# peterWon/LVI-ExC

Measured on AMD Instinct MI355X. Metric: M residual+Jacobian evals/s per GN iter, higher is better.
Workload: dtype f64; 1 GPU; config4-full-LVI: 1000000 surfel + 200000 IMU samples (gyro+accel blocks) + 49992 ORB reprojection blocks, 25023 knots @ dt=0.02; step = residuals + analytic Jacobians + Huber + J^T J/J^T r assembly (no linear solve); n_tangent=155259, bandwidth=179, n_border=52, tracks=orb, parallelism=sequence-per-gpu x1, allreduce_transport=none (one sequence)

## Files before the change

lvi-exc_amd/csrc/lvx_eval.hip:

```cpp
#include <algorithm>
#include <cmath>
#include <cstring>
#include <functional>
#include <numeric>
#include <cstdlib>

#include <thread>
#include "lvx_ctx.h"

namespace lvx {

#define LVX_PW 4
struct Keys { int k0, k1, lm; };
LVX_HD bool same(const Keys& a, const Keys& b) { return a.k0 == b.k0 && a.k1 == b.k1 && a.lm == b.lm; }

struct Cal { ImuCal imu; SensorCal lidar, cam; const double* rho; };
__device__ __forceinline__ Cal load_cal(const DevCommon& cm) {
  const double* s = cm.state + 7 * (size_t)cm.N;
  Cal c;
  c.imu.tau = s[7]; c.imu.roll = s[8]; c.imu.pitch = s[9]; c.imu.ba = load_v3(s + 10); c.imu.bg = load_v3(s + 13);
  c.lidar.q = load_q(s + 16); c.lidar.p = load_v3(s + 20); c.lidar.tau = s[23];
  c.cam.q = load_q(s + 24); c.cam.p = load_v3(s + 28); c.cam.tau = s[31];
  c.rho = s + 32;
  return c;
}

struct HubShared { PoseEval A; int ok; double M[6][24]; };

struct GyroFam {
  enum { NC = GYRO_NC, NR = GYRO_NR, USES_HUB = 0, FAM = LVX_FAM_GYRO, KEYS = 1 };
  int n; const double* t; const double* m3; const int* perm; double weight, huber;
  __device__ void make_hub(const DevCommon&, const SplineRef&, const Cal&, HubShared*) const {}
  __device__ int eval(const DevCommon& cm, const SplineRef& sp, const Cal& cal, const HubShared&, int si, double r[NR], double (*J)[NC], Keys& k) const {
    k.k1 = 0; k.lm = 0;
    return gyro_residual<true>(sp, cal.imu, t[si], load_v3(m3 + 3 * (size_t)si), weight, &k.k0, r, J);
  }
  __device__ int col(int c, const Keys& k, int N) const { return gyro_col(c, k.k0, N); }
};
struct AccelFam {
  enum { NC = ACC_NC, NR = ACC_NR, USES_HUB = 0, FAM = LVX_FAM_ACCEL, KEYS = 1 };
  int n; const double* t; const double* m3; const int* perm; double weight, huber;
// ... 312 lines not shown
    const int l0 = seg_l0[sg];
    const int l1 = sg + 1 < nseg ? seg_l0[sg + 1] : 64;
    const int rb = l0 * NR, re = l1 * NR;
    const int* cp = &cpos[sg * NC];
#pragma unroll
    for (int i = 0; i < ITER; ++i) {
      const int p = tid + NT * i;
      if (p < NP) {
        const int a = code[i] & 0xff, b = code[i] >> 8;
        const int pa = cp[a], pb = cp[b];
        if (pa == LVX_DEAD || pb == LVX_DEAD) continue;
        const double* ja = &Jt[a * TS];
        const double* jb = &Jt[b * TS];
        double acc = 0.0;
        for (int row = rb; row < re; ++row) acc += ja[row] * jb[row];
        if (a != b && pa == pb) acc *= 2.0;
        add_H(cm, pa, pb, acc, rep);
      } else if (p < NP + NC) {
        const int c = p - NP;
        const int pc = cp[c];
        if (pc == LVX_DEAD) continue;
        const double* jc = &Jt[c * TS];
        double acc = 0.0;
        for (int row = rb; row < re; ++row) acc += jc[row] * rs[row];
        add_g(cm, pc, acc, rep);
      }
    }
  }
}

__device__ void hub_eval_thread(const DevCommon& cm, double t_map, int want_surf, int want_cs, HubShared* hubs, int s) {
  if (s > 1) return;
  if ((s == 0 && !want_surf) || (s == 1 && !want_cs)) { hubs[s].ok = 0; return; }
  const SplineRef sp{cm.t0, cm.dt, cm.N, cm.state, cm.state + 3 * (size_t)cm.N};
  const Cal cal = load_cal(cm);
  const bool tl = s == 0 ? (cm.locks & LVX_LOCK_LIDAR_TAU) != 0 : (cm.locks & LVX_LOCK_CAM_TAU) != 0;
  const double tau = s == 0 ? cal.lidar.tau : cal.cam.tau;
  double s1[1][2]; hub_spans(t_map, tl, cm.sensor_mto, s1);
  Segs sg; KnotRef kh; hubs[s].ok = 0;
  if (!build_segments(sp, s1, 1, &sg)) return;
  if (!seg_lookup(sp, sg, t_map + tau, &kh)) return;
  if (!(tl ? pose_eval<true>(sp, kh, &hubs[s].A) : pose_eval<true, true>(sp, kh, &hubs[s].A))) { hubs[s].ok = -RES_NONUNIT; return; }
  hub_matrix(hubs[s].A, hubs[s].M);
  hubs[s].ok = 1;
}
__device__ __forceinline__ void state_prepass_block(const DevCommon& cm, So3Pre* tab, int nblk_tab, double t_map, int want_surf, int want_cs, HubShared* hubs, int blk) {
  if (blk >= nblk_tab) { hub_eval_thread(cm, t_map, want_surf, want_cs, hubs, threadIdx.x); return; }
  const int k = blk * blockDim.x + threadIdx.x;
  if (k >= cm.N) return;
  const double* so3 = cm.state + 3 * (size_t)cm.N;
  So3Pre e;
  if (k + 1 < cm.N) so3_pre(load_q(so3 + 4 * (size_t)k), load_q(so3 + 4 * (size_t)(k + 1)), &e);
  else { e.Om = mk(0, 0, 0); e.on = 0.0; e.Jri = m3_identity(); e.c3 = 1.0 / 12.0; e.ok = 1; }
  tab[k] = e;
}

struct Aux { int wid, xk, lm; const PreWin* pw; };
struct GyroAcc {
  enum { PMAJ = 1 };
  enum { NK = 12, NG = 3, NR = 3, HUB = -1, KPK = 3, LVO = 3, WS = 1, GL = 32, SKIP_GG = 0, SECONDARY = 0, LB = 64, NCP = 15, USE_PRE = 1, OCC = 1, FAM = LVX_FAM_GYRO };
  __device__ static constexpr int jm(int c) { return c; }
  int n; const double* t; const double* m3; const int* perm; double weight, huber;
  __device__ int eval(const DevCommon& cm, const SplineRef& sp, const Cal& cal, const HubShared*, int si, double r[NR], double (*J)[NCP], int& key, Aux& aux) const {
    return gyro_residual<true, true>(sp, cal.imu, t[si], load_v3(m3 + 3 * (size_t)si), weight, &key, r, J, aux.pw);
  }
  __device__ static int klv(int c) { return 6 * (c / 3) + 3 + c % 3; }
  __device__ static int gcol(int g, int N, int nt) { return 6 * N + 5 + g; }
  __device__ void put(const DevCommon& cm, const HubShared*, int si, bool valid, int key, const double (*J)[NCP]) const {
    if (!valid) { put_skipped(cm, FAM, perm[si]); return; }
    put_record<NR, GYRO_NC>(cm, FAM, perm[si], key, -1, -1, [&](int a, int c) { return J[a][c]; });
  }
};
#ifndef LVX_SURF_WS
#define LVX_SURF_WS 3
#endif
template <bool TAU> struct SurfAccT {
  enum { DEPG = LVX_SURF_WS >= 3 ? 3 : 0 };
// ... 1308 lines not shown
  const HubShared* hub = ((const HubShared*)cm.hubs) + set;
  if (hub->ok != 1) return;
  __shared__ double M[6][24];
  __shared__ int hrow[24];
  if (threadIdx.x < 144) M[threadIdx.x / 24][threadIdx.x % 24] = hub->M[threadIdx.x / 24][threadIdx.x % 24];
  if (threadIdx.x < 24) { const int o = cm.ord[6 * (hub->A.k.i0 + threadIdx.x / 6) + threadIdx.x % 6]; hrow[threadIdx.x] = (o != LVX_DEAD && o < 0) ? -1 - o : -1; }
  __syncthreads();
  const int j = blk * blockDim.x + threadIdx.x;
  double P[6];
  bool any = false;
  if (j < cm.nb) {
#pragma unroll
    for (int p = 0; p < 6; ++p) { P[p] = cm.Bd[(size_t)(cm.nbd_solve + 6 * set + p) * cm.nb + j]; any = any || P[p] != 0.0; }
  }
  const bool far = store && j < cm.nb && (j < cm.hub_lo || j >= cm.hub_hi);
  if (any || far) {
#pragma unroll
    for (int c = 0; c < 24; ++c) {
      if (hrow[c] < 0) continue;
      double s = 0.0;
#pragma unroll
      for (int p = 0; p < 6; ++p) s += M[p][c] * P[p];
      double* dst = &cm.Bd[(size_t)hrow[c] * cm.nb + j];
      if (far) *dst = any ? s : 0.0; else *dst += s;
    }
  }
  __syncthreads();
}
__global__ __launch_bounds__(256) void k_fold_border_rows(DevCommon cm, int set, int store) { fold_border_rows_block(cm, set, (int)blockIdx.x, store != 0); }
__device__ __forceinline__ void fold_border_dense_block(const DevCommon& cm) {
  extern __shared__ double Cf[];
  const int n = cm.nbd;
  double* g = Cf + n * n;
  for (int e0 = threadIdx.x; e0 < n * n; e0 += 8 * 256) {
    double v[8];
#pragma unroll
    for (int q = 0; q < 8; ++q) { const int e = e0 + 256 * q; if (e < n * n) { const int a = e / n, b = e % n; v[q] = a >= b ? cm.C[(size_t)a * n + b] : cm.C[(size_t)b * n + a]; } }
#pragma unroll
    for (int q = 0; q < 8; ++q) { const int e = e0 + 256 * q; if (e < n * n) Cf[e] = v[q]; }
  }
  for (int e = threadIdx.x; e < n; e += 256) g[e] = cm.gc[e];
  __syncthreads();
  for (int set = 0; set < 2; ++set) {
    const HubShared* hub = ((const HubShared*)cm.hubs) + set;
    if (hub->ok != 1) continue;
    __shared__ double M[6][24];
    __shared__ int hrow[24];
    if (threadIdx.x < 144) M[threadIdx.x / 24][threadIdx.x % 24] = hub->M[threadIdx.x / 24][threadIdx.x % 24];
    if (threadIdx.x < 24) { const int o = cm.ord[6 * (hub->A.k.i0 + threadIdx.x / 6) + threadIdx.x % 6]; hrow[threadIdx.x] = (o != LVX_DEAD && o < 0) ? -1 - o : -1; }
    __syncthreads();
    const int p0 = cm.nbd_solve + 6 * set;
    for (int e = threadIdx.x; e < 24 * n; e += 256) {
      const int c = e / n, col = e % n;
      if (hrow[c] < 0) continue;
      double s = 0.0;
      for (int p = 0; p < 6; ++p) s += M[p][c] * Cf[(p0 + p) * n + col];
      Cf[hrow[c] * n + col] += s;
    }
    if (threadIdx.x < 24 && hrow[threadIdx.x] >= 0) { double s = 0.0; for (int p = 0; p < 6; ++p) s += M[p][threadIdx.x] * g[p0 + p]; g[hrow[threadIdx.x]] += s; }
    __syncthreads();
    for (int e = threadIdx.x; e < 24 * n; e += 256) {
      const int c = e / n, row = e % n;
      if (hrow[c] < 0) continue;
      double s = 0.0;
      for (int p = 0; p < 6; ++p) s += Cf[row * n + p0 + p] * M[p][c];
      Cf[row * n + hrow[c]] += s;
    }
    __syncthreads();
  }
  for (int e = threadIdx.x; e < n * n; e += 256) { const int a = e / n, b = e % n; if (a >= b) cm.C[(size_t)a * n + b] = Cf[e]; }
  for (int e = threadIdx.x; e < n; e += 256) cm.gc[e] = g[e];
}

__global__ __launch_bounds__(256) void k_fold_border_dense(DevCommon cm) { fold_border_dense_block(cm); }

__device__ __forceinline__ double strided_sum(const double* p, size_t stride, int n) {
  double s = 0.0;
  for (int r0 = 0; r0 < n; r0 += 16) {
    double v[16];
#pragma unroll
    for (int q = 0; q < 16; ++q) v[q] = r0 + q < n ? p[(size_t)(r0 + q) * stride] : 0.0;
#pragma unroll
    for (int q = 0; q < 16; ++q) s += v[q];
  }
  return s;
}
__device__ __forceinline__ void fold_replicas_block(const DevCommon& cm, int blk) {
  const int n2 = cm.nbd * cm.nbd;
  const int i = blk * blockDim.x + threadIdx.x;
  if (cm.what & LVX_EVAL_NORMAL_EQ) {
    if (i < n2) cm.C[i] = strided_sum(cm.C + i, (size_t)n2, cm.nrep);
    if (i < cm.nbd) cm.gc[i] = strided_sum(cm.gc + i, (size_t)cm.nbd, cm.nrep);
  }
  if (i == 0) cm.cost[0] = strided_sum(cm.cost, 1, cm.nrep);
}
__global__ void k_fold_replicas(DevCommon cm) { fold_replicas_block(cm, (int)blockIdx.x); }
__global__ __launch_bounds__(256) void k_fold_all(DevCommon cm, int n_rep, int n_rows, int set0, int store0, int set1, int store1, int* ticket) {
  __shared__ int s_last;
  const int b = blockIdx.x;
  if (b < n_rep) {
    fold_replicas_block(cm, b);
    __threadfence();
    __syncthreads();
    if (threadIdx.x == 0) { const int t = atomicAdd(ticket, 1); s_last = t == n_rep - 1; if (s_last) *ticket = 0; }
    __syncthreads();
    if (!s_last) return;
    __threadfence();
    fold_border_dense_block(cm);
    return;
  }
  const int r = b - n_rep;
  fold_border_rows_block(cm, set0, r, store0 != 0);
  if (set1 >= 0) fold_border_rows_block(cm, set1, r, store1 != 0);
}
int fail(lvx_ctx* ctx, int code, const std::string& msg) { if (ctx) ctx->last_error = msg; return code; }

int dev_alloc(lvx_ctx* ctx, DevBuf& b, size_t bytes) {
  if (bytes == 0) bytes = 8;
  if (b.p && b.bytes >= bytes) return LVX_OK;
  if (b.p) { (void)hipFree(b.p); b.p = nullptr; b.bytes = 0; }
  if (hipMalloc(&b.p, bytes) != hipSuccess) { b.p = nullptr; return fail(ctx, LVX_E_ALLOC, "hipMalloc failed"); }
  b.bytes = bytes;
  return LVX_OK;
}
int upload(lvx_ctx* ctx, DevBuf& b, const void* src, size_t bytes) {
  int rc = dev_alloc(ctx, b, bytes);
  if (rc) return rc;
  if (bytes) LVX_HIP(ctx, hipMemcpyAsync(b.p, src, bytes, hipMemcpyHostToDevice, ctx->stream));
  return LVX_OK;
}
int upload_tmp(lvx_ctx* ctx, DevBuf& b, const void* src, size_t bytes) {
  int rc = upload(ctx, b, src, bytes);
  if (rc) return rc;
  LVX_HIP(ctx, hipStreamSynchronize(ctx->stream));
  return LVX_OK;
}

namespace {

template <class F> void par_for(size_t n, F&& fn) {
  const unsigned hw = std::thread::hardware_concurrency();
  const size_t nt = n < 200000 ? 1 : std::min<size_t>(8, hw ? hw : 1);
  if (nt <= 1) { fn((size_t)0, n); return; }
  std::vector<std::thread> th;
  const size_t per = (n + nt - 1) / nt;
  for (size_t t = 1; t < nt; ++t) { const size_t a = std::min(n, t * per), b = std::min(n, a + per); if (a < b) th.emplace_back([&fn, a, b] { fn(a, b); }); }
// ... 637 lines not shown
        double* col = bc.Hb + (size_t)j * bc.ld;
        if (!(bc.ld & 1)) {
          uint4* c4 = (uint4*)col;
          for (int e = (beg >> 1) + l16; e < (len >> 1); e += 16) c4[e] = make_uint4(0u, 0u, 0u, 0u);
          if ((len & 1) && l16 == 0 && len > beg) col[len - 1] = 0.0;
        } else {
          for (int e = beg + l16; e < len; e += 16) col[e] = 0.0;
        }
      }
      if (bc.own && !owned) {
        if (l16 == 8) bc.gb[j] = 0.0;
        else if (l16 < 8 && ((bc.imu_rows >> l16) & 1u)) bc.Bd_imu[(size_t)l16 * bc.nb + j] = 0.0;
      }
    }
    return;
  }
  if ((int)blockIdx.x < npre + bc.nblk + bc.hub_blk) {
    const int row = (int)blockIdx.x - npre - bc.nblk;
    double* dst = bc.Bd + (size_t)row * bc.nb;
    for (int e = bc.hub_lo + threadIdx.x; e < bc.hub_hi; e += blockDim.x) dst[e] = 0.0;
    return;
  }
  const int first = npre + bc.nblk + bc.hub_blk;
  const size_t stride = (size_t)(gridDim.x - first) * blockDim.x, t0 = (size_t)(blockIdx.x - first) * blockDim.x + threadIdx.x;
  for (int b = 0; b < cl.n; ++b) {
    const size_t nw = cl.words[b];
    size_t i = t0;
    for (; i + 3 * stride < nw; i += 4 * stride) {
      cl.p[b][i] = make_uint4(0u, 0u, 0u, 0u); cl.p[b][i + stride] = make_uint4(0u, 0u, 0u, 0u);
      cl.p[b][i + 2 * stride] = make_uint4(0u, 0u, 0u, 0u); cl.p[b][i + 3 * stride] = make_uint4(0u, 0u, 0u, 0u);
    }
    for (; i < nw; i += stride) cl.p[b][i] = make_uint4(0u, 0u, 0u, 0u);
  }
}

template <class F, int PW>
static void launch_family(bool exp, dim3 grid, dim3 block, hipStream_t s, const F& f, const DevCommon& cm, const uint16_t* pairs, long long row0, const int* rows = nullptr, const int* nrows = nullptr) {
  if (exp) hipLaunchKernelGGL((k_family<F, PW, true>), grid, block, 0, s, f, cm, pairs, row0, rows, nrows);
  else hipLaunchKernelGGL((k_family<F, PW>), grid, block, 0, s, f, cm, pairs, row0, rows, nrows);
}
static GyroFam gyro_fam(const lvx_ctx* c) { const Family& f = c->imu; return {f.n, (const double*)f.d_t.p, (const double*)f.d_a3.p, (const int*)f.d_perm.p, f.weight, 0.0}; }
static GyroAcc gyro_acc(const lvx_ctx* c) { const Family& f = c->imu; return {f.n, (const double*)f.d_t.p, (const double*)f.d_a3.p, (const int*)f.d_perm.p, f.weight, 0.0}; }
static AccelFam accel_fam(const lvx_ctx* c) { const Family& f = c->imu; return {f.n, (const double*)f.d_t.p, (const double*)f.d_b3.p, (const int*)f.d_perm.p, f.huber , 0.0}; }
static ImuFused imu_fused(const lvx_ctx* c) { const Family& f = c->imu; return {f.n, (const double*)f.d_t.p, (const double*)f.d_a3.p, (const double*)f.d_b3.p, (const int*)f.d_perm.p, f.weight, f.huber }; }
static PriorFam prior_fam(const lvx_ctx* c) { return {1, c->prior_t, mkq(c->prior_q[0], c->prior_q[1], c->prior_q[2], c->prior_q[3]), (const int*)c->d_zero.p, c->prior_w, 0.0}; }
template <bool TAU> static SurfFamT<TAU> surf_fam(const lvx_ctx* c) { const Family& f = c->surf; return {f.n, (const double*)f.d_t.p, (const double*)f.d_a3.p, (const int*)f.d_id0.p, (const int*)f.d_perm.p, (const double*)c->d_planes.p, c->t_map, f.weight, f.huber}; }
template <bool TAU> static SurfAccT<TAU> surf_acc(const lvx_ctx* c) { const Family& f = c->surf; return {f.n, (const double*)f.d_t.p, (const double*)f.d_a3.p, (const double*)f.d_b3.p, (const int*)f.d_perm.p, c->t_map, f.weight, f.huber}; }
template <bool TAU> static CamSurfFamT<TAU> camsurf_fam(const lvx_ctx* c) { const Family& f = c->cs; return {f.n, (const int*)f.d_id0.p, (const int*)f.d_id1.p, (const int*)f.d_perm.p, (const double*)c->d_planes.p, (const double*)c->d_lm_uv.p, (const double*)c->d_lm_t0.p, c->t_map, f.weight, f.huber}; }
template <bool TAU> static CamSurfAccT<TAU> camsurf_acc(const lvx_ctx* c) { const Family& f = c->cs; return {f.n, (const int*)f.d_id0.p, (const int*)f.d_id1.p, (const int*)f.d_perm.p, (const double*)c->d_planes.p, (const double*)c->d_lm_uv.p, (const double*)c->d_lm_t0.p, c->t_map, f.weight, f.huber}; }
template <bool TAU> static ReprojFamT<TAU> reproj_fam(const lvx_ctx* c) { const Family& f = c->rep; return {f.n, (const int*)f.d_id0.p, (const double*)f.d_a3.p, (const double*)f.d_t.p, (const int*)f.d_perm.p, (const double*)c->d_lm_uv.p, (const double*)c->d_lm_t0.p, f.weight, f.huber}; }
template <bool TAU> static LidarPosFamT<TAU> lidarpos_fam(const lvx_ctx* c) { const Family& f = c->lp; return {f.n, (const double*)f.d_t.p, (const double*)f.d_a3.p, (const int*)f.d_perm.p, c->lp_t_start, f.weight, f.huber}; }
static int setup_blocks(lvx_ctx* ctx, DevCommon& cm) {
  static const int nrs[LVX_NUM_FAM] = {GYRO_NR, ACC_NR, PRI_NR, SURF_NR, REP_NR, CS_NR};
  const bool tauL = !(ctx->locks & LVX_LOCK_LIDAR_TAU), tauC = !(ctx->locks & LVX_LOCK_CAM_TAU);
  int64_t nk = 0, nv = 0;
  for (int f = 0; f < LVX_NUM_FAM; ++f) {
    ctx->xb_nr[f] = nrs[f];
    ctx->xb_w[f] = block_width(f, f == LVX_FAM_SURFEL ? tauL : (f >= LVX_FAM_REPROJ ? tauC : false));
    ctx->xb_n[f] = (ctx->fam_row0[f + 1] - ctx->fam_row0[f]) / nrs[f];
    ctx->xb_off[f] = nk; ctx->xb_voff[f] = nv;
    nk += ctx->xb_n[f]; nv += ctx->xb_n[f] * nrs[f] * ctx->xb_w[f];
  }
  int rc;
  if ((rc = dev_alloc(ctx, ctx->d_xkeys, (size_t)std::max<int64_t>(nk, 1) * 12))) return rc;
  if ((rc = dev_alloc(ctx, ctx->d_xvals, (size_t)std::max<int64_t>(nv, 1) * 8))) return rc;
  if (ctx->h_xkeys_cap < (size_t)nk * 3) {
// ... 43 lines not shown
    }
    LVX_HIP(ctx, hipEventRecord(ctx->ev_xb[f], s_cp));
    return LVX_OK;
  }
  static dim3 grid(int n) { return dim3((unsigned)((n + 63) / 64)); }
};
static Pass make_pass(lvx_ctx* ctx, const DevCommon& cm, uint32_t what) {
  Pass p{}; p.ctx = ctx; p.cm = cm; p.what = what; p.xb = (what & LVX_EVAL_JACOBIAN_BLOCKS) != 0;
  p.fast = !ctx->force_legacy && !(what & LVX_EVAL_JACOBIAN) && !ctx->sw.force_legacy; p.fb = ctx->fb_on && p.fast;
  p.det = ctx->sw.deterministic != 0; p.side_on = !ctx->sw.serial && !p.det;
  p.tauL = !(ctx->locks & LVX_LOCK_LIDAR_TAU); p.tauC = !(ctx->locks & LVX_LOCK_CAM_TAU);
  p.fast_surf = p.fast && ctx->surf.n > 0; p.fast_cs = p.fast && ctx->cs.n > 0;
  p.imu_fused_on = p.fast && ctx->imu.n > 0 && !(ctx->locks & LVX_LOCK_R3) && ctx->imu_nch > 0 && imu_fused_lds_bytes(ctx->imu_span) <= 160 * 1024;
  p.imu_own = p.imu_fused_on && (what & LVX_EVAL_NORMAL_EQ) && ctx->nb > 0 && ctx->imu_owned_cols > 0 && !ctx->sw.clear_all;
  p.st = ctx->stream; p.s_fb = p.side_on ? ctx->fam_stream[1] : p.st; p.s_side = p.side_on ? ctx->fam_stream[0] : p.st; p.s_cp = ctx->fam_stream[2];
  return p;
}
template <class FT, int OCC, bool EXP> static int launch_mfma_occ(Pass& p, const FT& fam, int chunk_slot, hipStream_t stream, long long row0) {
  lvx_ctx* ctx = p.ctx; const size_t lds = mfma_lds_bytes<FT>(ctx->chunk_r[chunk_slot]);
  LVX_HIP(ctx, hipFuncSetAttribute((const void*)k_family_mfma<FT, OCC, EXP>, hipFuncAttributeMaxDynamicSharedMemorySize, (int)lds));
  const int* chunks = (const int*)ctx->d_chunk[chunk_slot].p; const int cr = ctx->chunk_r[chunk_slot], nvar = ctx->chunk_var[chunk_slot] ? ctx->n_chunk[chunk_slot] : 0;
  const std::vector<int>& dc = ctx->det_col[chunk_slot];
  if (p.det && dc.size() > 1) {
    for (size_t q = 0; q + 1 < dc.size(); ++q)
      hipLaunchKernelGGL((k_family_mfma<FT, OCC, EXP>), dim3(dc[q + 1] - dc[q]), dim3(256), lds, stream, fam, p.cm, chunks, row0, cr, nvar, (const int*)ctx->d_det_list[chunk_slot].p + dc[q]);
  } else
    hipLaunchKernelGGL((k_family_mfma<FT, OCC, EXP>), dim3(ctx->n_chunk[chunk_slot]), dim3(256), lds, stream, fam, p.cm, chunks, row0, cr, nvar, (const int*)nullptr);
  return LVX_OK;
}
template <class FT> static int launch_mfma(Pass& p, const FT& fam, int chunk_slot, hipStream_t stream, long long row0) {
  if constexpr ((int)FT::OCC == 1) return p.xb ? launch_mfma_occ<FT, 1, true>(p, fam, chunk_slot, stream, row0) : launch_mfma_occ<FT, 1, false>(p, fam, chunk_slot, stream, row0);
  else return p.xb ? launch_mfma_occ<FT, 2, true>(p, fam, chunk_slot, stream, row0) : launch_mfma_occ<FT, 2, false>(p, fam, chunk_slot, stream, row0);
}
template <class F, int PW> static void launch_family_list(Pass& p, int f, int list, hipStream_t s, const F& fam) {
  launch_family<F, PW>(p.xb, dim3((unsigned)(LVX_FB_CAP / 64)) , dim3(64 * PW), s, fam, p.cm, (const uint16_t*)p.ctx->d_pairs[f].p, (long long)p.ctx->fam_row0[f], p.fb_rows(list), p.fb_cnt(list));
}
template <class F, int PW> static void launch_family_all(Pass& p, int f, const F& fam) {
  launch_family<F, PW>(p.xb, Pass::grid(fam.n), dim3(64 * PW), p.st, fam, p.cm, (const uint16_t*)p.ctx->d_pairs[f].p, (long long)p.ctx->fam_row0[f]);
}
template <class Fn> static int with_tau(bool tau, Fn&& fn) { return tau ? fn(std::true_type{}) : fn(std::false_type{}); }
static int step_clear(Pass& p) {
  lvx_ctx* ctx = p.ctx; DevCommon& cm = p.cm; const uint32_t what = p.what; hipStream_t st = p.st;
  const bool fast = p.fast, fb = p.fb, fast_surf = p.fast_surf, fast_cs = p.fast_cs, imu_own = p.imu_own;
  const int nblk_tab = fast ? (ctx->N + 255) / 256 : 0, npre = fast ? nblk_tab + ((fast_surf || fast_cs) ? 1 : 0) : 0;
  ClearList cl{}; BandClear bc{};
  auto add = [&](void* ptr, size_t bytes) { if (cl.n < 16) { cl.p[cl.n] = (uint4*)ptr; cl.words[cl.n] = (bytes + 15) / 16; cl.n++; } };
  add(cm.cost, (size_t)ctx->nrep * 8); add(cm.err, 64);
  if (what & LVX_EVAL_NORMAL_EQ) {
    const size_t nb1 = (size_t)std::max(ctx->nb, 1);
    if (ctx->sw.clear_all || ctx->nb == 0) add(cm.Hb, nb1 * (ctx->bw + 1) * 8);
    else { bc.Hb = cm.Hb; bc.colfull = (const uint8_t*)ctx->d_colfull.p; bc.nb = ctx->nb; bc.ld = ctx->bw + 1; bc.npre = ctx->clear_npre; bc.nblk = std::min((ctx->nb + 15) / 16, 2048); }
    if (imu_own) {
      bc.own = (const int*)ctx->d_imu_own.p; bc.gb = cm.gb; bc.Bd_imu = cm.Bd + (size_t)6 * ctx->n_hub * nb1; bc.imu_rows = 0;
      for (int c = 0; c < 8; ++c) if (ctx->bd_row_live[6 * ctx->n_hub + c]) bc.imu_rows |= 1u << c;
      if (!bc.nblk) { bc.colfull = (const uint8_t*)ctx->d_colfull.p; bc.nb = ctx->nb; bc.ld = ctx->bw + 1; bc.npre = ctx->clear_npre; bc.nblk = std::min((ctx->nb + 15) / 16, 2048); }
    } else add(cm.gb, nb1 * 8);
    const bool fb_lidar = fb && (ctx->fb_mask & ((1 << LVX_FAM_SURFEL) | (1 << LVX_FAM_CAMSURF)));
    const bool hub_partial = !fb_lidar && ctx->lp.n <= 0 && !ctx->sw.clear_all && !(nb1 & 1) && ctx->nb > 0 && ctx->n_hub > 0 && (fast_surf || fast_cs) && (ctx->surf.n == 0 || fast_surf) && (ctx->cs.n == 0 || fast_cs);
    cm.hub_lo = hub_partial ? ctx->hub_near_lo : 0; cm.hub_hi = hub_partial ? ctx->hub_near_hi : ctx->nb;
    if (hub_partial) { bc.Bd = cm.Bd; bc.hub_rows = 6 * ctx->n_hub; bc.hub_lo = cm.hub_lo; bc.hub_hi = cm.hub_hi; bc.hub_blk = cm.hub_hi > cm.hub_lo ? 6 * ctx->n_hub : 0; if (!bc.nb) bc.nb = ctx->nb; }
    if (ctx->sw.clear_all || (nb1 & 1)) add(cm.Bd, (size_t)ctx->nbd_ext * nb1 * 8);
    else for (int b0 = 0; b0 < ctx->nbd_ext;) {
      const int first_live = hub_partial ? 6 * ctx->n_hub : 0;
      const int imu0 = imu_own ? 6 * ctx->n_hub : -1;
      if (b0 < first_live || !ctx->bd_row_live[b0] || (imu0 >= 0 && b0 >= imu0 && b0 < imu0 + 8)) { ++b0; continue; }
      int b1 = b0; while (b1 < ctx->nbd_ext && ctx->bd_row_live[b1] && !(imu0 >= 0 && b1 >= imu0 && b1 < imu0 + 8)) ++b1;
      add(cm.Bd + (size_t)b0 * nb1, (size_t)(b1 - b0) * nb1 * 8);
// ... 30 lines not shown
  }
  if (ctx->imu.n <= 0) return LVX_OK;
  if (p.fast) {
    ProfScope ps(ctx, LVX_FAM_GYRO, st);
    if ((rc = launch_mfma(p, gyro_acc(ctx), LVX_FAM_GYRO, st, ctx->fam_row0[0]))) return rc;
    if (listed) { if ((rc = p.fb_fork())) return rc;
      ProfScope psf(ctx, LVX_KERNEL_FIXUP, p.s_fb);
      launch_family_list<GyroFam, 1>(p, LVX_FAM_GYRO, LVX_FAM_GYRO, p.s_fb, gyro_fam(ctx));
    }
  } else {
    ProfScope ps(ctx, LVX_FAM_GYRO, st);
    launch_family_all<GyroFam, 1>(p, LVX_FAM_GYRO, gyro_fam(ctx));
  }
  if (!(ctx->locks & LVX_LOCK_R3)) {
    ProfScope ps(ctx, LVX_FAM_ACCEL, st);
    launch_family_all<AccelFam, LVX_PW>(p, LVX_FAM_ACCEL, accel_fam(ctx));
  }
  return (rc = p.xb_copy(LVX_FAM_GYRO, listed ? p.s_fb : st)) ? rc : p.xb_copy(LVX_FAM_ACCEL, st);
}
static int step_prior(Pass& p) {
  if (!p.ctx->has_prior) return LVX_OK;
  ProfScope ps(p.ctx, LVX_FAM_PRIOR, p.st);
  launch_family<PriorFam, 1>(p.xb, dim3(1), dim3(64), p.st, prior_fam(p.ctx), p.cm, (const uint16_t*)p.ctx->d_pairs[2].p, (long long)p.ctx->fam_row0[2]);
  return p.xb_copy(LVX_FAM_PRIOR, p.st);
}
template <class Acc, class Fam> static int step_lidar(Pass& p, int f, bool fused, const Acc& acc, const Fam& fam) {
  lvx_ctx* ctx = p.ctx; int rc;
  const bool listed = fused && p.fb_fam(f);
  ProfScope ps(ctx, f, p.st);
  if (fused) {
    if ((rc = launch_mfma(p, acc, f, p.st, ctx->fam_row0[f]))) return rc;
    if (listed) { if ((rc = p.fb_fork())) return rc;
      ProfScope psf(ctx, LVX_KERNEL_FIXUP, p.s_fb);
      launch_family_list<Fam, LVX_PW>(p, f, f, p.s_fb, fam);
    }
  } else launch_family_all<Fam, 1>(p, f, fam);
  return p.xb_copy(f, listed ? p.s_fb : p.st);
}
static int step_surfel(Pass& p) {
  return p.ctx->surf.n <= 0 ? LVX_OK : with_tau(p.tauL, [&](auto T) { return step_lidar(p, LVX_FAM_SURFEL, p.fast_surf, surf_acc<decltype(T)::value>(p.ctx), surf_fam<decltype(T)::value>(p.ctx)); });
}
static int step_camsurf(Pass& p) {
  return p.ctx->cs.n <= 0 ? LVX_OK : with_tau(p.tauC, [&](auto T) { return step_lidar(p, LVX_FAM_CAMSURF, p.fast_cs, camsurf_acc<decltype(T)::value>(p.ctx), camsurf_fam<decltype(T)::value>(p.ctx)); });
}
static int step_lidarpos(Pass& p) {
  lvx_ctx* ctx = p.ctx;
  if (ctx->lp.n <= 0) return LVX_OK;
  return with_tau(p.tauL, [&](auto T) {
    using F = LidarPosFamT<decltype(T)::value>;
    ProfScope ps(ctx, LVX_KERNEL_LIDAR_POS, p.st);
    hipLaunchKernelGGL((k_family<F, LVX_PW>), Pass::grid(ctx->lp.n), dim3(64 * LVX_PW), 0, p.st, lidarpos_fam<decltype(T)::value>(ctx), p.cm, (const uint16_t*)ctx->d_pairs_lp.p, (long long)ctx->fam_row0[LVX_NUM_FAM]);
    return (int)LVX_OK;
  });
}
template <bool T> static int rep_fused(Pass& p) {
  lvx_ctx* ctx = p.ctx; hipStream_t st = p.st; int rc;
  constexpr int RJ = REP_NC + (T ? 1 : 0);
  const ReprojFamT<T> rf = reproj_fam<T>(ctx);
  double* Jb = (double*)ctx->d_repB[0].p; double* rb = Jb + (size_t)2 * RJ * rf.n; int* kb = (int*)ctx->d_repB[1].p;
  { ProfScope ps(ctx, LVX_KERNEL_REP_JAC, st);
    double* trec = (ctx->L > 0 && !(ctx->locks & LVX_LOCK_LANDMARKS) && ctx->rep_groups > 0 && (p.what & LVX_EVAL_NORMAL_EQ)) ? (double*)ctx->d_repT.p : (double*)nullptr;
    const size_t lds_j = trec ? (size_t)64 * ((56 + (T ? 1 : 0)) | 1) * 8 : 0;
    if (p.xb) hipLaunchKernelGGL((k_reproj_jac<T, true>), Pass::grid(rf.n), dim3(64), lds_j, st, rf, p.cm, Jb, rb, kb, (long long)ctx->fam_row0[4], trec);
    else hipLaunchKernelGGL(k_reproj_jac<T>, Pass::grid(rf.n), dim3(64), lds_j, st, rf, p.cm, Jb, rb, kb, (long long)ctx->fam_row0[4], trec); }
  if (!p.fb_fam(LVX_FAM_REPROJ) && (rc = p.xb_copy(LVX_FAM_REPROJ, st))) return rc;
  if (!(p.what & LVX_EVAL_NORMAL_EQ)) return LVX_OK;
  const RepJac jac{Jb, rb, kb, rf.n};
// ... 20 lines not shown
    const RepLmRows lq{(const double*)ctx->d_repT.p, kb, rf.n, lp, lp + ctx->L + 1, ctx->L};
    const size_t lds = (size_t)4 * ctx->lm_ls * 8;
    LVX_HIP(ctx, hipFuncSetAttribute((const void*)k_reproj_lmrows<T>, hipFuncAttributeMaxDynamicSharedMemorySize, (int)lds));
    ProfScope ps(ctx, LVX_KERNEL_REP_LMROWS, st);
    hipLaunchKernelGGL(k_reproj_lmrows<T>, dim3((unsigned)((ctx->L + 3) / 4)), dim3(256), lds, st, lq, p.cm);
  }
  return LVX_OK;
}
template <bool T> static int rep_one(Pass& p) {
  lvx_ctx* ctx = p.ctx;
  const int* tab = (const int*)ctx->d_repF.p; const int ng = ctx->rep_fused_wg;
  const RepFused q{tab, tab + ng, ng};
  ProfScope ps(ctx, LVX_KERNEL_REP_FUSED, p.st);
  hipLaunchKernelGGL(k_reproj_fused<T>, dim3((unsigned)std::min((ng + 3) / 4, ctx->n_cu)), dim3(256), 0, p.st, reproj_fam<T>(ctx), q, p.cm, (long long)ctx->fam_row0[4]);
  return LVX_OK;
}
template <bool T> static int step_reproj_tau(Pass& p) {
  lvx_ctx* ctx = p.ctx; int rc;
  if (!p.fast) {
    { ProfScope ps(ctx, LVX_FAM_REPROJ, p.st); launch_family_all<ReprojFamT<T>, LVX_PW>(p, LVX_FAM_REPROJ, reproj_fam<T>(ctx)); }
    return p.xb_copy(LVX_FAM_REPROJ, p.st);
  }
  if ((rc = (ctx->rep_fused_wg > 0 && !p.xb) ? rep_one<T>(p) : rep_fused<T>(p))) return rc;
  if (!p.fb_fam(LVX_FAM_REPROJ)) return LVX_OK;
  { ProfScope psf(ctx, LVX_KERNEL_FIXUP, p.st); launch_family_list<ReprojFamT<T>, LVX_PW>(p, LVX_FAM_REPROJ, LVX_FAM_REPROJ, p.st, reproj_fam<T>(ctx)); }
  return p.xb_copy(LVX_FAM_REPROJ, p.st);
}
static int step_reproj(Pass& p) { return p.ctx->rep.n <= 0 ? LVX_OK : with_tau(p.tauC, [&](auto T) { return step_reproj_tau<decltype(T)::value>(p); }); }
static int step_fold(Pass& p) {
  lvx_ctx* ctx = p.ctx; hipStream_t st = p.st; const DevCommon& cm = p.cm; const bool fast_surf = p.fast_surf, fast_cs = p.fast_cs;
  ProfScope ps(ctx, LVX_KERNEL_FOLD);
  const bool fold_fast = (p.what & LVX_EVAL_NORMAL_EQ) && (fast_surf || fast_cs);
  const unsigned n_rep_blk = (unsigned)((ctx->nbd_ext * ctx->nbd_ext + 255) / 256);
  if (fold_fast && ctx->nb > 0 && !ctx->sw.serial) {
    const unsigned n_rows_blk = (unsigned)((ctx->nb + 255) / 256);
    const int set0 = fast_surf ? 0 : 1, set1 = (fast_surf && fast_cs) ? 1 : -1;
    const size_t lds = ((size_t)ctx->nbd_ext * ctx->nbd_ext + ctx->nbd_ext) * 8;
    LVX_HIP(ctx, hipFuncSetAttribute((const void*)k_fold_all, hipFuncAttributeMaxDynamicSharedMemorySize, (int)lds));
    hipLaunchKernelGGL(k_fold_all, dim3(n_rep_blk + n_rows_blk), dim3(256), lds, st, cm, (int)n_rep_blk, (int)n_rows_blk, set0, 1, set1, 0, (int*)ctx->d_zero.p + 1);
    return LVX_OK;
  }
  hipStream_t s_fold = (fold_fast && p.side_on) ? ctx->fam_stream[0] : st;
  if (s_fold != st) { LVX_HIP(ctx, hipEventRecord(ctx->ev_fork, st)); LVX_HIP(ctx, hipStreamWaitEvent(s_fold, ctx->ev_fork, 0)); }
  hipLaunchKernelGGL(k_fold_replicas, dim3(n_rep_blk), dim3(256), 0, st, cm);
  if (fold_fast) {
    for (int set = 0; set < 2; ++set) if (ctx->nb > 0 && ((set == 0 && fast_surf) || (set == 1 && fast_cs)))
      hipLaunchKernelGGL(k_fold_border_rows, dim3((unsigned)((ctx->nb + 255) / 256)), dim3(256), 0, s_fold, cm, set, (set == 0 || !fast_surf) ? 1 : 0);
    const size_t lds = ((size_t)ctx->nbd_ext * ctx->nbd_ext + ctx->nbd_ext) * 8;
    LVX_HIP(ctx, hipFuncSetAttribute((const void*)k_fold_border_dense, hipFuncAttributeMaxDynamicSharedMemorySize, (int)lds));
    hipLaunchKernelGGL(k_fold_border_dense, dim3(1), dim3(256), lds, st, cm);
    if (s_fold != st) { LVX_HIP(ctx, hipEventRecord(ctx->ev_join[1], s_fold)); LVX_HIP(ctx, hipStreamWaitEvent(st, ctx->ev_join[1], 0)); }
  }
  return LVX_OK;
}
static int enqueue_pass(Pass& p) {
  lvx_ctx* ctx = p.ctx; int rc;
  if ((rc = step_clear(p)) || (rc = step_imu(p)) || (rc = step_prior(p)) || (rc = step_surfel(p)) || (rc = step_camsurf(p)) || (rc = step_lidarpos(p)) || (rc = step_reproj(p))) return rc;
  if (p.side_used) { LVX_HIP(ctx, hipEventRecord(ctx->ev_join[0], p.s_side)); LVX_HIP(ctx, hipStreamWaitEvent(p.st, ctx->ev_join[0], 0)); }
  if (p.fb_used) { LVX_HIP(ctx, hipEventRecord(ctx->ev_join[2], p.s_fb)); LVX_HIP(ctx, hipStreamWaitEvent(p.st, ctx->ev_join[2], 0)); }
  if ((rc = step_fold(p))) return rc;
  LVX_HIP(ctx, hipGetLastError());
  return LVX_OK;
}
static int finish_pass_errors(lvx_ctx* ctx, const int* errw, bool* rerun) {
  *rerun = false;
  ctx->fallback_rows = 0; for (int f = 0; f < LVX_NUM_FAM; ++f) ctx->fallback_rows += errw[4 + f];
  if ((errw[0] & LVX_ERR_FALLBACK) && !ctx->force_legacy) {
    int need = 0; for (int f = 0; f < LVX_NUM_FAM; ++f) if (errw[4 + f] > 0) need |= 1 << f;
    if (!ctx->sw.force_legacy && need && (need & ~ctx->fb_mask)) { ctx->fb_on = true; ctx->fb_mask |= need; }
    else ctx->force_legacy = true;
    *rerun = true; return LVX_OK;
  }
// ... 91 lines not shown
```

Before: 2796 Mevals/s.

## Fold border dense block in closed form across replica-sum blocks

Replaces the single-workgroup serial dense border fold, which ran after the replica reduction, with a closed-form fold. Each replica-sum block now computes its own entries, C + U^T R + R^T U + U^T R_pp U, from the hub rows. A separate block folds the gradient and cost, and the last block through the ticket fixes up the pseudo rows. This is meant to remove the serial tail where one 256-thread workgroup staged the whole n×n matrix in LDS. It adds redundant hub-row strided sums in every block and a 64-wide unrolled load. It also adds timing printfs behind a macro and a deterministic fallback-row sort for the det mode.

```diff
diff --git a/lvi-exc_amd/csrc/lvx_eval.hip b/lvi-exc_amd/csrc/lvx_eval.hip
--- a/lvi-exc_amd/csrc/lvx_eval.hip
+++ b/lvi-exc_amd/csrc/lvx_eval.hip
@@ -7,6 +7,7 @@
 
 #include <thread>
 #include "lvx_ctx.h"
+#include "lvx_fold.h"
 
 namespace lvx {
 
@@ -385,17 +386,31 @@
 __device__ void hub_eval_thread(const DevCommon& cm, double t_map, int want_surf, int want_cs, HubShared* hubs, int s) {
   if (s > 1) return;
   if ((s == 0 && !want_surf) || (s == 1 && !want_cs)) { hubs[s].ok = 0; return; }
+#ifdef LVX_KTIME_FOLD
+  long long kt_[5] = {0, 0, 0, 0, 0}; long long kt0_ = __builtin_amdgcn_s_memtime(); const long long kts_ = kt0_;
+#define HKT(i) { const long long n_ = __builtin_amdgcn_s_memtime(); kt_[i] += n_ - kt0_; kt0_ = n_; }
+#else
+#define HKT(i)
+#endif
   const SplineRef sp{cm.t0, cm.dt, cm.N, cm.state, cm.state + 3 * (size_t)cm.N};
   const Cal cal = load_cal(cm);
   const bool tl = s == 0 ? (cm.locks & LVX_LOCK_LIDAR_TAU) != 0 : (cm.locks & LVX_LOCK_CAM_TAU) != 0;
   const double tau = s == 0 ? cal.lidar.tau : cal.cam.tau;
   double s1[1][2]; hub_spans(t_map, tl, cm.sensor_mto, s1);
+  HKT(0)
   Segs sg; KnotRef kh; hubs[s].ok = 0;
   if (!build_segments(sp, s1, 1, &sg)) return;
   if (!seg_lookup(sp, sg, t_map + tau, &kh)) return;
+  HKT(1)
   if (!(tl ? pose_eval<true>(sp, kh, &hubs[s].A) : pose_eval<true, true>(sp, kh, &hubs[s].A))) { hubs[s].ok = -RES_NONUNIT; return; }
+  HKT(2)
   hub_matrix(hubs[s].A, hubs[s].M);
   hubs[s].ok = 1;
+  HKT(3)
+#ifdef LVX_KTIME_FOLD
+  printf("HKT hub set %d: cal+spans %lld segments+lookup %lld pose_eval %lld hub_matrix+stores %lld | total %lld, ends at %lld (ticks of s_memtime)\n", s, kt_[0], kt_[1], kt_[2], kt_[3],
+         (long long)__builtin_amdgcn_s_memtime() - kts_, (long long)__builtin_amdgcn_s_memtime());
+#endif
 }
 __device__ __forceinline__ void state_prepass_block(const DevCommon& cm, So3Pre* tab, int nblk_tab, double t_map, int want_surf, int want_cs, HubShared* hubs, int blk) {
   if (blk >= nblk_tab) { hub_eval_thread(cm, t_map, want_surf, want_cs, hubs, threadIdx.x); return; }
@@ -1770,6 +1785,12 @@
   extern __shared__ double Cf[];
   const int n = cm.nbd;
   double* g = Cf + n * n;
+#ifdef LVX_KTIME_FOLD
+  long long kt_[4] = {0, 0, 0, 0}; long long kt0_ = __builtin_amdgcn_s_memtime(); const long long kts_ = kt0_;
+#define DKT(i) { const long long n_ = __builtin_amdgcn_s_memtime(); kt_[i] += n_ - kt0_; kt0_ = n_; }
+#else
+#define DKT(i)
+#endif
   for (int e0 = threadIdx.x; e0 < n * n; e0 += 8 * 256) {
     double v[8];
 #pragma unroll
@@ -1779,6 +1800,7 @@
   }
   for (int e = threadIdx.x; e < n; e += 256) g[e] = cm.gc[e];
   __syncthreads();
+  DKT(0)
   for (int set = 0; set < 2; ++set) {
     const HubShared* hub = ((const HubShared*)cm.hubs) + set;
     if (hub->ok != 1) continue;
@@ -1797,6 +1819,7 @@
     }
     if (threadIdx.x < 24 && hrow[threadIdx.x] >= 0) { double s = 0.0; for (int p = 0; p < 6; ++p) s += M[p][threadIdx.x] * g[p0 + p]; g[hrow[threadIdx.x]] += s; }
     __syncthreads();
+    DKT(1)
     for (int e = threadIdx.x; e < 24 * n; e += 256) {
       const int c = e / n, row = e % n;
       if (hrow[c] < 0) continue;
@@ -1805,9 +1828,14 @@
       Cf[row * n + hrow[c]] += s;
     }
     __syncthreads();
+    DKT(2)
   }
   for (int e = threadIdx.x; e < n * n; e += 256) { const int a = e / n, b = e % n; if (a >= b) cm.C[(size_t)a * n + b] = Cf[e]; }
   for (int e = threadIdx.x; e < n; e += 256) cm.gc[e] = g[e];
+  DKT(3)
+#ifdef LVX_KTIME_FOLD
+  if (threadIdx.x == 0) printf("FKT dense block (one workgroup, n %d): load %lld rows %lld columns %lld store %lld | total %lld\n", n, kt_[0], kt_[1], kt_[2], kt_[3], (long long)__builtin_amdgcn_s_memtime() - kts_);
+#endif
 }
 
 __global__ __launch_bounds__(256) void k_fold_border_dense(DevCommon cm) { fold_border_dense_block(cm); }
@@ -1833,23 +1861,102 @@
   if (i == 0) cm.cost[0] = strided_sum(cm.cost, 1, cm.nrep);
 }
 __global__ void k_fold_replicas(DevCommon cm) { fold_replicas_block(cm, (int)blockIdx.x); }
+__device__ __forceinline__ double strided_sum64(const double* p, size_t stride, int n) {
+  double s = 0.0;
+  for (int r0 = 0; r0 < n; r0 += 64) {
+    double v[64];
+#pragma unroll
+    for (int q = 0; q < 64; ++q) v[q] = r0 + q < n ? p[(size_t)(r0 + q) * stride] : 0.0;
+#pragma unroll
+    for (int q = 0; q < 64; ++q) s += v[q];
+  }
+  return s;
+}
+#define LVX_FOLD_OWN 128
+__device__ __forceinline__ void fold_load_U(const DevCommon& cm, unsigned want, double* U, int n) {
+  for (int s = 0; s < 2; ++s) {
+    const HubShared* hub = ((const HubShared*)cm.hubs) + s;
+    if (!((want >> s) & 1u) || hub->ok != 1) continue;
+    if (threadIdx.x < 144) {
+      const int p = threadIdx.x / 24, c = threadIdx.x % 24;
+      const int o = cm.ord[6 * (hub->A.k.i0 + c / 6) + c % 6];
+      if (o != LVX_DEAD && o < 0) U[(6 * s + p) * n + (-1 - o)] = hub->M[p][c];
+    }
+  }
+}
+__device__ __forceinline__ void fold_dense_closed_block(const DevCommon& cm, int blk, int n_rep, int set0, int set1, int* ticket) {
+  extern __shared__ double Lf[];
+  __shared__ int s_last;
+  const int n = cm.nbd, pp = cm.nbd_solve, n2 = n * n, tid = threadIdx.x;
+  double* R = Lf; double* U = Lf + 12 * n;
+#ifdef LVX_KTIME_FOLD
+  long long kt_[6] = {0, 0, 0, 0, 0, 0}; long long kt0_ = __builtin_amdgcn_s_memtime(); const long long kts_ = kt0_;
+#define FKT(i) { const long long n_ = __builtin_amdgcn_s_memtime(); kt_[i] += n_ - kt0_; kt0_ = n_; }
+#else
+#define FKT(i)
+#endif
+  const unsigned want = (1u << set0) | (set1 >= 0 ? 1u << set1 : 0u);
+  for (int e = tid; e < 24 * n + 12; e += 256) Lf[e] = 0.0;
+  __syncthreads();
+  fold_load_U(cm, want, U, n);
+  const int i = tid >= 256 - LVX_FOLD_OWN ? blk * LVX_FOLD_OWN + tid - (256 - LVX_FOLD_OWN) : n2, a = i / n, b = i % n;
+  const bool own = i < n2 && !(a >= b && a >= pp && ((want >> ((a - pp) / 6)) & 1u));
+  const double S = own ? strided_sum64(cm.C + i, (size_t)n2, cm.nrep) : 0.0;
+  const int k_first = set1 >= 0 ? 0 : 6 * set0, n_items = (set1 >= 0 ? 12 : 6) * n;
+  for (int e = tid; e < n_items; e += 256) {
+    const int k = k_first + e / n, x = e % n;
+    if (x > pp + k) continue;
+    const double v = strided_sum64(cm.C + (size_t)(pp + k) * n + x, (size_t)n2, cm.nrep);
+    R[k * n + x] = v;
+    if (x >= pp && x != pp + k) R[(x - pp) * n + pp + k] = v;
+  }
+  FKT(0)
+  __threadfence();
+  __syncthreads();
+  if (tid == 0) { const int t = atomicAdd(ticket, 1); s_last = t == n_rep - 1; if (s_last) *ticket = 0; }
+  FKT(1)
+  if (own) cm.C[i] = a >= b ? fold_dense_entry(a, b, S, R, U, n, pp) : S;
+  FKT(2)
+  __syncthreads();
+  if (s_last) {
+    for (int e = tid; e < n_items; e += 256) {
+      const int k = k_first + e / n, x = e % n;
+      if (x <= pp + k) cm.C[(size_t)(pp + k) * n + x] = fold_dense_entry(pp + k, x, R[k * n + x], R, U, n, pp);
+    }
+  }
+  FKT(3)
+#ifdef LVX_KTIME_FOLD
+  if (tid == 0 && (blk == 0 || blk == n_rep - 1 || s_last))
+    printf("FKT fold replica blk %d last %d: sums+rows %lld ticket %lld own %lld pseudo %lld | total %lld (ticks of s_memtime)\n", blk, s_last, kt_[0], kt_[1], kt_[2], kt_[3], (long long)__builtin_amdgcn_s_memtime() - kts_);
+#endif
+}
+__device__ __forceinline__ void fold_grad_block(const DevCommon& cm, int set0, int set1) {
+  extern __shared__ double Lf[];
+  const int n = cm.nbd, pp = cm.nbd_solve, j = threadIdx.x;
+  double* U = Lf + 12 * n; double* gp = Lf + 24 * n;
+  for (int e = j; e < 12 * n + 12; e += 256) U[e] = 0.0;
+  __syncthreads();
+  fold_load_U(cm, (1u << set0) | (set1 >= 0 ? 1u << set1 : 0u), U, n);
+  double Sg = 0.0;
+  if (j <= n) Sg = j < n ? strided_sum64(cm.gc + j, (size_t)n, cm.nrep) : strided_sum64(cm.cost, 1, cm.nrep);
+  if (j >= pp && j < n) gp[j - pp] = Sg;
+  __syncthreads();
+  if (j < n) cm.gc[j] = fold_dense_grad(j, Sg, gp, U, n);
+  else if (j == n) cm.cost[0] = Sg;
+}
 __global__ __launch_bounds__(256) void k_fold_all(DevCommon cm, int n_rep, int n_rows, int set0, int store0, int set1, int store1, int* ticket) {
-  __shared__ int s_last;
   const int b = blockIdx.x;
-  if (b < n_rep) {
-    fold_replicas_block(cm, b);
-    __threadfence();
-    __syncthreads();
-    if (threadIdx.x == 0) { const int t = atomicAdd(ticket, 1); s_last = t == n_rep - 1; if (s_last) *ticket = 0; }
-    __syncthreads();
-    if (!s_last) return;
-    __threadfence();
-    fold_border_dense_block(cm);
-    return;
-  }
-  const int r = b - n_rep;
+  if (b < n_rep) { fold_dense_closed_block(cm, b, n_rep, set0, set1, ticket); return; }
+  if (b == n_rep) { fold_grad_block(cm, set0, set1); return; }
+  const int r = b - n_rep - 1;
+#ifdef LVX_KTIME_FOLD
+  const long long kts_ = __builtin_amdgcn_s_memtime();
+#endif
   fold_border_rows_block(cm, set0, r, store0 != 0);
   if (set1 >= 0) fold_border_rows_block(cm, set1, r, store1 != 0);
+#ifdef LVX_KTIME_FOLD
+  if (threadIdx.x == 0 && (r == 0 || r == n_rows / 2 || r == n_rows - 1)) printf("FKT fold border-row blk %d of %d: total %lld\n", r, n_rows, (long long)__builtin_amdgcn_s_memtime() - kts_);
+#endif
 }
 int fail(lvx_ctx* ctx, int code, const std::string& msg) { if (ctx) ctx->last_error = msg; return code; }
 
@@ -2553,6 +2660,9 @@
     }
     for (; i < nw; i += stride) cl.p[b][i] = make_uint4(0u, 0u, 0u, 0u);
   }
+#ifdef LVX_KTIME_FOLD
+  if (blockIdx.x == gridDim.x - 1 && threadIdx.x == 0) printf("HKT k_clear: last clear block (%u) ends at %lld\n", blockIdx.x, (long long)__builtin_amdgcn_s_memtime());
+#endif
 }
 
 template <class F, int PW>
@@ -2662,7 +2772,20 @@
   if constexpr ((int)FT::OCC == 1) return p.xb ? launch_mfma_occ<FT, 1, true>(p, fam, chunk_slot, stream, row0) : launch_mfma_occ<FT, 1, false>(p, fam, chunk_slot, stream, row0);
   else return p.xb ? launch_mfma_occ<FT, 2, true>(p, fam, chunk_slot, stream, row0) : launch_mfma_occ<FT, 2, false>(p, fam, chunk_slot, stream, row0);
 }
+__global__ __launch_bounds__(256) void k_fb_sort(int* rows, const int* nrows, int cap) {
+  __shared__ int a[LVX_FB_CAP];
+  const int n = min(*nrows, min(cap, LVX_FB_CAP));
+  for (int i = threadIdx.x; i < n; i += 256) a[i] = rows[i];
+  __syncthreads();
+  for (int i = threadIdx.x; i < n; i += 256) {
+    const int v = a[i];
+    int r = 0;
+    for (int j = 0; j < n; ++j) r += (a[j] < v || (a[j] == v && j < i)) ? 1 : 0;
+    rows[r] = v;
+  }
+}
 template <class F, int PW> static void launch_family_list(Pass& p, int f, int list, hipStream_t s, const F& fam) {
+  if (p.det) hipLaunchKernelGGL(k_fb_sort, dim3(1), dim3(256), 0, s, const_cast<int*>(p.fb_rows(list)), p.fb_cnt(list), LVX_FB_CAP);
   launch_family<F, PW>(p.xb, dim3((unsigned)(LVX_FB_CAP / 64)) , dim3(64 * PW), s, fam, p.cm, (const uint16_t*)p.ctx->d_pairs[f].p, (long long)p.ctx->fam_row0[f], p.fb_rows(list), p.fb_cnt(list));
 }
 template <class F, int PW> static void launch_family_all(Pass& p, int f, const F& fam) {
@@ -2759,7 +2882,8 @@
     if ((rc = launch_mfma(p, acc, f, p.st, ctx->fam_row0[f]))) return rc;
     if (listed) { if ((rc = p.fb_fork())) return rc;
       ProfScope psf(ctx, LVX_KERNEL_FIXUP, p.s_fb);
-      launch_family_list<Fam, LVX_PW>(p, f, f, p.s_fb, fam);
+      if (p.det) launch_family_list<Fam, 1>(p, f, f, p.s_fb, fam);
+      else launch_family_list<Fam, LVX_PW>(p, f, f, p.s_fb, fam);
     }
   } else launch_family_all<Fam, 1>(p, f, fam);
   return p.xb_copy(f, listed ? p.s_fb : p.st);
@@ -2846,12 +2970,12 @@
   ProfScope ps(ctx, LVX_KERNEL_FOLD);
   const bool fold_fast = (p.what & LVX_EVAL_NORMAL_EQ) && (fast_surf || fast_cs);
   const unsigned n_rep_blk = (unsigned)((ctx->nbd_ext * ctx->nbd_ext + 255) / 256);
-  if (fold_fast && ctx->nb > 0 && !ctx->sw.serial) {
+  if (fold_fast && ctx->nb > 0 && !ctx->sw.serial && ctx->nbd_ext <= 255) {
     const unsigned n_rows_blk = (unsigned)((ctx->nb + 255) / 256);
     const int set0 = fast_surf ? 0 : 1, set1 = (fast_surf && fast_cs) ? 1 : -1;
-    const size_t lds = ((size_t)ctx->nbd_ext * ctx->nbd_ext + ctx->nbd_ext) * 8;
-    LVX_HIP(ctx, hipFuncSetAttribute((const void*)k_fold_all, hipFuncAttributeMaxDynamicSharedMemorySize, (int)lds));
-    hipLaunchKernelGGL(k_fold_all, dim3(n_rep_blk + n_rows_blk), dim3(256), lds, st, cm, (int)n_rep_blk, (int)n_rows_blk, set0, 1, set1, 0, (int*)ctx->d_zero.p + 1);
+    const size_t lds = ((size_t)2 * LVX_FOLD_NP * ctx->nbd_ext + LVX_FOLD_NP) * 8;
+    const unsigned n_dense_blk = (unsigned)((ctx->nbd_ext * ctx->nbd_ext + LVX_FOLD_OWN - 1) / LVX_FOLD_OWN);
+    hipLaunchKernelGGL(k_fold_all, dim3(n_dense_blk + 1 + n_rows_blk), dim3(256), lds, st, cm, (int)n_dense_blk, (int)n_rows_blk, set0, 1, set1, 0, (int*)ctx->d_zero.p + 1);
     return LVX_OK;
   }
   hipStream_t s_fold = (fold_fast && p.side_on) ? ctx->fam_stream[0] : st;
diff --git a/lvi-exc_amd/csrc/lvx_fold.h b/lvi-exc_amd/csrc/lvx_fold.h
--- /dev/null
+++ b/lvi-exc_amd/csrc/lvx_fold.h
@@ -0,0 +1,30 @@
+#pragma once
+#include "lvx_math.h"
+
+namespace lvx {
+
+#define LVX_FOLD_NP 12
+
+LVX_HD double fold_dense_entry(int a, int b, double S, const double* R, const double* U, int n, int pp) {
+  double ua[LVX_FOLD_NP], ub[LVX_FOLD_NP], ra[LVX_FOLD_NP], rb[LVX_FOLD_NP];
+  bool hub_a = false, hub_b = false;
+  for (int k = 0; k < LVX_FOLD_NP; ++k) { ua[k] = U[k * n + a]; ub[k] = U[k * n + b]; ra[k] = R[k * n + a]; rb[k] = R[k * n + b]; hub_a = hub_a || ua[k] != 0.0; hub_b = hub_b || ub[k] != 0.0; }
+  double v = S;
+  for (int k = 0; k < LVX_FOLD_NP; ++k) v = ua[k] != 0.0 ? v + ua[k] * rb[k] : v;
+  for (int k = 0; k < LVX_FOLD_NP; ++k) v = ub[k] != 0.0 ? v + ra[k] * ub[k] : v;
+  if (hub_a && hub_b) {
+    for (int k = 0; k < LVX_FOLD_NP; ++k) {
+      double t = 0.0;
+      for (int l = 0; l < LVX_FOLD_NP; ++l) t = ub[l] != 0.0 ? t + R[k * n + pp + l] * ub[l] : t;
+      v = ua[k] != 0.0 ? v + ua[k] * t : v;
+    }
+  }
+  return v;
+}
+LVX_HD double fold_dense_grad(int x, double S, const double* gp, const double* U, int n) {
+  double v = S;
+  for (int k = 0; k < LVX_FOLD_NP; ++k) { const double u = U[k * n + x]; if (u != 0.0) v += u * gp[k]; }
+  return v;
+}
+
+}
```

Result: faster. 2849 Mevals/s (median of 6 runs) (+1.9%).
